# BaeHann/feature_level_style_transfer_for_TSC

Hardware: AMD Instinct MI355X
Metric: train-step samples/sec (univariate TS, len=512, batch=256) at 1/2/4/8 MI355X (higher is better)
Workload: dtype bf16x3

## Files before the change

### feature_level_style_transfer_for_tsc_amd/_lib.py

```python
from __future__ import annotations

import ctypes
import os
from ctypes import POINTER, Structure, c_char_p, c_float, c_int, c_int32, c_int64, c_void_p
from typing import Optional

import torch

ABI_VERSION = 13
_LIB_NAME = "libfst_hip.so"
_HERE = os.path.dirname(os.path.abspath(__file__))
LIB_PATH = os.environ.get("FST_HIP_LIB", os.path.join(_HERE, _LIB_NAME))


class FstLibraryError(RuntimeError):
    pass


class WSrc(Structure):
    _fields_ = [("w", c_void_p), ("off0", c_int64), ("sm", c_int64), ("sc", c_int64), ("st", c_int64)]


_P = c_void_p
_I32P = c_void_p
_SIGNATURES = {
    "fst_version": (c_int, []),
    "fst_last_error": (c_char_p, []),
    "fst_pack_weights": (c_int, [_I32P, _I32P, c_int, POINTER(WSrc), POINTER(WSrc), c_int, c_int, c_int, c_int, _P, c_void_p]),
    "fst_pack_weights_bf16x3": (c_int, [_I32P, _I32P, c_int, POINTER(WSrc), POINTER(WSrc), c_int, c_int, c_int, c_int, _P, c_void_p]),
    "fst_unpack_weights": (c_int, [_I32P, _I32P, c_int, _P, c_int, _P, c_int64, c_int64, c_int64, c_int64,
                                   _P, c_int64, c_int64, c_int64, c_int64, c_int, c_void_p]),
    "fst_mask_taps": (c_int, [_P, _I32P, _I32P, c_int, c_int, c_int, c_void_p]),
    "fst_conv_gemm": (c_int, [_P, c_int64, _P, c_int64, _P, _I32P, _I32P, c_int, _P, _P, c_int64, _P, c_int64,
                              _P, c_int64, c_int, c_int, c_int, c_int, c_int, c_int, c_int, c_int, c_void_p]),
    "fst_conv_wgrad": (c_int, [_P, c_int64, _P, c_int64, _P, c_int64, _P, c_int64, c_int, _P, _I32P, _I32P, c_int,
                               c_int, c_int, c_int, c_int, c_int, c_int64, c_void_p]),
    "fst_conv_last_route": (c_int, [POINTER(c_int32)]),
    "fst_row_sum": (c_int, [_P, c_int64, c_int, c_int, c_int, _P, c_void_p]),
    "fst_bn_stats": (c_int, [_P, c_int, c_int, c_int, _P, c_int64, c_void_p]),
    "fst_bn_finalize": (c_int, [_P, c_int, _P, _P, _P, _P, c_int, c_int, c_float, c_float, _P, c_void_p]),
    "fst_bn_apply": (c_int, [_P, _P, _P, _P, _P, c_int, c_int, c_int, c_int, c_int64, c_void_p]),
    "fst_bn_bwd_reduce": (c_int, [_P, _P, _P, _P, c_int, c_int, c_int, c_int, _P, c_int64, c_void_p]),
    "fst_bn_bwd_apply": (c_int, [_P, _P, _P, _P, _P, c_int, _P, _P, _P, c_int, c_int, c_int, c_int, c_int, c_int, c_int64, c_void_p]),
    "fst_gate_fwd": (c_int, [_P, _P, c_int, c_int, c_int, c_int64, c_void_p]),
    "fst_gate_bwd": (c_int, [_P, _P, _P, c_int, c_int, c_int, c_int64, c_void_p]),
    "fst_coupling_sum_slots": (c_int64, [c_int, c_int, c_int]),
    "fst_coupling_fwd": (c_int, [_P, _P, _P, c_int, c_int, c_int, c_int64, _P, c_void_p]),
    "fst_coupling_bwd": (c_int, [_P, _P, _P, _P, _P, _P, _P, _P, c_int, c_int, c_int, c_int64, c_void_p]),
    "fst_coupling_inv_fwd": (c_int, [_P, _P, _P, c_int, c_int, c_int, c_int64, c_void_p]),
    "fst_coupling_inv_bwd": (c_int, [_P, _P, _P, _P, _P, c_int, c_int, c_int, c_int64, c_void_p]),
    "fst_rmsprop_multi": (c_int, [_P, _P, _P, _P, _P, c_int, c_float, c_float, c_void_p]),
    "fst_adam_multi": (c_int, [_P, _P, _P, _P, _P, c_int, _P, c_float, c_float, c_float, c_float, c_void_p]),
    "fst_wn_stack_fwd_ok": (c_int, [c_int, c_int, c_int, c_int]),
    "fst_wn_stack_fwd": (c_int, [_P, _P, _P, c_int64, _P, _P, _P, c_int64, _P, c_int, c_int, c_int, c_int, c_int, c_int64, c_void_p]),
    "fst_wn_stack_bwd_ok": (c_int, [c_int, c_int, c_int, c_int]),
    "fst_wn_stack_bwd": (c_int, [_P, _P, _P, _P, _P, _P, _P, _P, _P, c_int64, c_int, c_int, c_int, c_int, c_int, c_int64, c_void_p]),
    "fst_wn_wgrad_ok": (c_int, [c_int, c_int, c_int, c_int, c_int, c_int]),
    "fst_wn_wgrad_workspace_floats": (c_int64, [c_int, c_int, c_int, c_int, c_int, c_int]),
    "fst_wn_wgrad_in": (c_int, [_P, _P, _P, c_int, c_int64, _P, _P, _P, c_int64, c_int, c_int, c_int, c_int, c_int, c_int, c_int64,
                                c_void_p]),
    "fst_wn_wgrad_rs": (c_int, [_P, _P, _P, c_int, _P, _P, c_int64, c_int, c_int, c_int, c_int, c_int64, c_void_p]),
    "fst_nt_gemm_workspace_floats": (c_int64, [c_int, c_int, c_int]),
    "fst_nt_gemm": (c_int, [_P, _P, _P, _P, c_int64, c_int, c_int, c_int, _P, _P, c_int, c_float, _P, c_void_p]),
    "fst_tap_wgrad_ok": (c_int, [c_int, c_int, c_int, c_int, c_int, c_int, c_int]),
    "fst_tap_wgrad_workspace_floats": (c_int64, [c_int, c_int, c_int, c_int, c_int]),
    "fst_tap_wgrad": (c_int, [_P, _P, _P, _P, c_int64, c_int, c_int, c_int, c_int, c_int, c_int, c_int, c_int, c_int64, c_int64, c_void_p]),
    "fst_dense_tap_wgrad_ok": (c_int, [c_int, c_int, c_int, c_int, c_int, c_int]),
    "fst_dense_tap_wgrad_workspace_floats": (c_int64, [c_int, c_int, c_int, c_int, c_int]),
    "fst_dense_tap_wgrad": (c_int, [_P, _P, _P, _P, c_int64, c_int, c_int, c_int, c_int, c_int, c_int, c_int64, c_int64, c_void_p]),
    "fst_relu_bwd": (c_int, [_P, _P, _P, c_int64, c_void_p]),
    "fst_gemm_workspace_floats": (c_int64, [c_int, c_int, c_int]),
    "fst_gemm": (c_int, [_P, c_int64, c_int, _P, c_int64, c_int, _P, c_int64, c_int, c_int, c_int, _P, c_int, c_float, _P, c_int64,
                         c_void_p]),
    "fst_act_bwd": (c_int, [_P, _P, _P, c_int64, c_float, c_void_p]),
    "fst_batch_sum": (c_int, [_P, _P, _P, c_int, c_int64, c_int, c_void_p]),
    "fst_noise_transfer_fwd": (c_int, [_P, c_int, c_int, _P, _P, c_float, c_float, _P, _P, _P, _P, _P, _P, _P, c_int, c_int, c_void_p]),
# ... 82 lines not shown
```

### feature_level_style_transfer_for_tsc_amd/csrc/pointwise.hip

```cpp
#include "fst_common.h"

static thread_local char g_err[512] = "";
void fst_set_error(const char* fmt, ...) {
  va_list ap;
  va_start(ap, fmt);
  vsnprintf(g_err, sizeof(g_err), fmt, ap);
  va_end(ap);
}
extern "C" const char* fst_last_error(void) { return g_err; }

int fst_allow_full_lds(const void* fn, const char* who) {
  static const void* done[64];
  static int n_done = 0;
  for (int i = 0; i < n_done; ++i)
    if (done[i] == fn) return 0;
  hipError_t e = hipFuncSetAttribute(fn, hipFuncAttributeMaxDynamicSharedMemorySize, 160 * 1024);
  if (e != hipSuccess) {
    fst_set_error("%s: hipFuncSetAttribute: %s", who, hipGetErrorString(e));
    return (int)e;
  }
  if (n_done < 64) done[n_done++] = fn;
  return 0;
}
int fst_cu_count(void) {
// ... 174 lines not shown
      const double nn = n + nb, d = mb - m;
      m += d * (nb / nn);
      m2 += Mb + d * d * (n * nb / nn);
      n = nn;
    }
    const double v = n > 0.0 ? m2 / n : 0.0;
    mean = (float)m;
    var = (float)v;
    const float unbiased = n > 1.0 ? (float)(m2 / (n - 1.0)) : var;
    rmean[c] = (1.f - momentum) * rmean[c] + momentum * mean;
    rvar[c] = (1.f - momentum) * rvar[c] + momentum * unbiased;
  } else {
    mean = rmean[c];
    var = rvar[c];
  }
  const float invstd = 1.0f / sqrtf(var + eps);
  const float scale = gamma[c] * invstd;
  stats[c] = mean;
  stats[C + c] = invstd;
  stats[2 * C + c] = scale;
  stats[3 * C + c] = beta[c] - mean * scale;
}

extern "C" int fst_bn_finalize(const float* part, int n_slots, const float* gamma, const float* beta, float* running_mean,
                               float* running_var, int train, int C, float eps, float momentum, float* stats, void* stream) {
  FST_REQUIRE(gamma && beta && running_mean && running_var && stats && C > 0, "fst_bn_finalize: bad arguments");
  FST_REQUIRE(!train || (part && n_slots > 0), "fst_bn_finalize: train mode needs the moment partials (n_slots=%d)", n_slots);
  hipLaunchKernelGGL(bn_finalize_kernel, dim3((C + 63) / 64), dim3(64), 0, (hipStream_t)stream, part, n_slots, gamma, beta,
                     running_mean, running_var, train, C, eps, momentum, stats);
  FST_LAUNCH_CHECK();
  return 0;
}

__global__ __launch_bounds__(256) void bn_apply_kernel(const float* y, const float* stats, const float* res,
                                                       const float* res_stats, float* out, int C, int L, int relu) {
  const int bc = blockIdx.x;
  const int c = bc % C;
  const float sc = stats[2 * C + c], sh = stats[3 * C + c];
  float rsc = 1.f, rsh = 0.f;
  if (res && res_stats) { rsc = res_stats[2 * C + c]; rsh = res_stats[3 * C + c]; }
  const long long base = (long long)bc * L;
  for (int t = threadIdx.x; t < L; t += 256) {
    float v = y[base + t] * sc + sh;
    if (res) v += res[base + t] * rsc + rsh;
    if (relu) v = fmaxf(v, 0.f);
    out[base + t] = v;
  }
}

__global__ __launch_bounds__(256) void bn_apply_vec_kernel(const float* y, const float* stats, const float* res,
                                                           const float* res_stats, float* out, int rows, int C, int L,
                                                           int relu, RowVec rv) {
  const int r = threadIdx.x >> rv.shift, t0 = threadIdx.x & ((1 << rv.shift) - 1), rpp = 256 >> rv.shift;
  const int bc = blockIdx.x * rpp + r;
  if (bc >= rows) return;
  const int c = bc % C;
  const float sc = stats[2 * C + c], sh = stats[3 * C + c];
  float rsc = 1.f, rsh = 0.f;
  if (res && res_stats) { rsc = res_stats[2 * C + c]; rsh = res_stats[3 * C + c]; }
  const long long base = (long long)bc * rv.L4;
  const float4* y4 = reinterpret_cast<const float4*>(y) + base;
  const float4* r4 = res ? reinterpret_cast<const float4*>(res) + base : nullptr;
  float4* o4 = reinterpret_cast<float4*>(out) + base;
  for (int t = t0; t < rv.L4; t += 1 << rv.shift) {
    float4 v = y4[t];
    v.x = v.x * sc + sh; v.y = v.y * sc + sh; v.z = v.z * sc + sh; v.w = v.w * sc + sh;
    if (r4) {
      const float4 q = r4[t];
      v.x += q.x * rsc + rsh; v.y += q.y * rsc + rsh; v.z += q.z * rsc + rsh; v.w += q.w * rsc + rsh;
    }
    if (relu) { v.x = fmaxf(v.x, 0.f); v.y = fmaxf(v.y, 0.f); v.z = fmaxf(v.z, 0.f); v.w = fmaxf(v.w, 0.f); }
    o4[t] = v;
  }
}

extern "C" int fst_bn_apply(const float* y, const float* stats, const float* res, const float* res_stats, float* out,
                            int B, int C, int L, int relu, int64_t numel, void* stream) {
  FST_REQUIRE(y && stats && out && B > 0 && C > 0 && L > 0, "fst_bn_apply: bad arguments");
  FST_REQUIRE_EXTENT("fst_bn_apply", B, C, L, numel);
  if (vec_ok(L, {y, res, out})) {
    const RowVec rv = row_vec(L);
    const int rpp = 256 >> rv.shift;
    hipLaunchKernelGGL(bn_apply_vec_kernel, dim3((B * C + rpp - 1) / rpp), dim3(256), 0, (hipStream_t)stream, y, stats, res,
                       res_stats, out, B * C, C, L, relu, rv);
  } else {
    hipLaunchKernelGGL(bn_apply_kernel, dim3(B * C), dim3(256), 0, (hipStream_t)stream, y, stats, res, res_stats, out, C, L, relu);
  }
  FST_LAUNCH_CHECK();
  return 0;
}

__global__ __launch_bounds__(256) void bn_bwd_reduce_kernel(const float* dy, const float* y, const float* out,
                                                            const float* stats, int B, int C, int L, int relu, float* red) {
  const int c = blockIdx.x;
  const float mean = stats[c], invstd = stats[C + c];
  float s1 = 0.f, s2 = 0.f;
  for (int b = blockIdx.y; b < B; b += gridDim.y) {
    const long long base = ((long long)b * C + c) * L;
    for (int t = threadIdx.x; t < L; t += 256) {
      float g = dy[base + t];
      if (relu && !(out[base + t] > 0.f)) g = 0.f;
      s1 += g;
// ... 54 lines not shown
}

__device__ __forceinline__ void bn_red_sums(const float* red, int n_slots, int C, int c, float& r1, float& r2) {
  r1 = 0.f; r2 = 0.f;
  for (int s = 0; s < n_slots; ++s) {
    r1 += red[(long long)c * n_slots + s];
    r2 += red[((long long)C + c) * n_slots + s];
  }
}

__global__ __launch_bounds__(256) void bn_bwd_apply_kernel(const float* dy, const float* y, const float* out,
                                                           const float* stats, const float* red, int n_slots, float* red_out,
                                                           float* dx, float* row_sums, int C, int L, int relu, int train, float invN) {
  const int bc = blockIdx.x;
  const int c = bc % C;
  const float mean = stats[c], invstd = stats[C + c], scale = stats[2 * C + c];
  float r1 = 0.f, r2 = 0.f;
  if (red) bn_red_sums(red, n_slots, C, c, r1, r2);
  if (red_out && bc < C && threadIdx.x == 0) { red_out[c] = r1; red_out[C + c] = r2; }
  const float m1 = train ? r1 * invN : 0.f, m2 = train ? r2 * invN : 0.f;
  const long long base = (long long)bc * L;
  float rs = 0.f, dummy = 0.f;
  for (int t = threadIdx.x; t < L; t += 256) {
    float g = dy[base + t];
    if (relu && !(out[base + t] > 0.f)) g = 0.f;
    const float xh = (y[base + t] - mean) * invstd;
    const float d = scale * (g - m1 - xh * m2);
    dx[base + t] = d;
    rs += d;
  }
  if (row_sums) {
    block_sum2(rs, dummy);
    if (threadIdx.x == 0) row_sums[bc] = rs;
  }
}

__global__ __launch_bounds__(256) void bn_bwd_apply_vec_kernel(const float* dy, const float* y, const float* out,
                                                               const float* stats, const float* red, int n_slots,
                                                               float* red_out, float* dx, float* row_sums, int rows, int C,
                                                               int L, int relu, int train, float invN, RowVec rv) {
  __shared__ float wsum[4];
  const int r = threadIdx.x >> rv.shift, t0 = threadIdx.x & ((1 << rv.shift) - 1), rpp = 256 >> rv.shift;
  const int bc_raw = blockIdx.x * rpp + r;
  const bool live = bc_raw < rows;
  const int bc = live ? bc_raw : rows - 1;
  const int c = bc % C;
  const float mean = stats[c], invstd = stats[C + c], scale = stats[2 * C + c];
  float r1 = 0.f, r2 = 0.f;
  if (red) bn_red_sums(red, n_slots, C, c, r1, r2);
  if (red_out && live && bc < C && t0 == 0) { red_out[c] = r1; red_out[C + c] = r2; }
  const float m1 = train ? r1 * invN : 0.f, m2 = train ? r2 * invN : 0.f;
  const long long base = (long long)bc * rv.L4;
  const float4* dy4 = reinterpret_cast<const float4*>(dy) + base;
  const float4* y4 = reinterpret_cast<const float4*>(y) + base;
  const float4* o4 = reinterpret_cast<const float4*>(out) + base;
  float4* dx4 = reinterpret_cast<float4*>(dx) + base;
  float rs = 0.f;
  for (int t = t0; t < rv.L4; t += 1 << rv.shift) {
    float4 g = dy4[t];
    const float4 v = y4[t];
    if (relu) {
      const float4 o = o4[t];
      if (!(o.x > 0.f)) g.x = 0.f;
      if (!(o.y > 0.f)) g.y = 0.f;
      if (!(o.z > 0.f)) g.z = 0.f;
      if (!(o.w > 0.f)) g.w = 0.f;
    }
    float4 d;
    d.x = scale * (g.x - m1 - (v.x - mean) * invstd * m2);
    d.y = scale * (g.y - m1 - (v.y - mean) * invstd * m2);
    d.z = scale * (g.z - m1 - (v.z - mean) * invstd * m2);
    d.w = scale * (g.w - m1 - (v.w - mean) * invstd * m2);
    if (live) dx4[t] = d;
    rs += (d.x + d.y) + (d.z + d.w);
  }
  if (row_sums) {
    const int w = rv.shift < 6 ? rv.shift : 6;
    for (int o = (1 << w) >> 1; o > 0; o >>= 1) rs += __shfl_xor(rs, o, 64);
    if (rv.shift <= 6) {
      if (live && t0 == 0) row_sums[bc] = rs;
    } else {
      if ((threadIdx.x & 63) == 0) wsum[threadIdx.x >> 6] = rs;
      __syncthreads();
      if (live && t0 == 0) {
        const int w0 = threadIdx.x >> 6, nw = 1 << (rv.shift - 6);
        float tot = 0.f;
        for (int i = 0; i < nw; ++i) tot += wsum[w0 + i];
        row_sums[bc] = tot;
      }
    }
  }
}

extern "C" int fst_bn_bwd_apply(const float* dy, const float* y, const float* out, const float* stats, const float* red,
                                int n_slots, float* red_out, float* dx, float* row_sums, int B, int C, int L, int relu, int train,
                                int B_total, int64_t numel, void* stream) {
  FST_REQUIRE(dy && y && stats && dx && (!relu || out) && (!train || red), "fst_bn_bwd_apply: bad arguments");
  FST_REQUIRE(B > 0 && C > 0 && L > 0 && B_total >= B, "fst_bn_bwd_apply: B=%d C=%d L=%d B_total=%d", B, C, L, B_total);
  FST_REQUIRE(!red || n_slots > 0, "fst_bn_bwd_apply: n_slots=%d", n_slots);
  FST_REQUIRE(!red_out || red, "fst_bn_bwd_apply: red_out needs red");
  FST_REQUIRE_EXTENT("fst_bn_bwd_apply", B, C, L, numel);
  if (vec_ok(L, {dy, y, out, dx})) {
    const RowVec rv = row_vec(L);
    const int rpp = 256 >> rv.shift;
    hipLaunchKernelGGL(bn_bwd_apply_vec_kernel, dim3((B * C + rpp - 1) / rpp), dim3(256), 0, (hipStream_t)stream, dy, y, out,
                       stats, red, n_slots, red_out, dx, row_sums, B * C, C, L, relu, train, 1.0f / ((float)B_total * (float)L), rv);
  } else {
    hipLaunchKernelGGL(bn_bwd_apply_kernel, dim3(B * C), dim3(256), 0, (hipStream_t)stream, dy, y, out, stats, red, n_slots,
                       red_out, dx, row_sums, C, L, relu, train, 1.0f / ((float)B_total * (float)L));
  }
  FST_LAUNCH_CHECK();
  return 0;
}

__global__ __launch_bounds__(256) void gate_fwd_kernel(float* g, float* acts, int n, int L) {
  const int b = blockIdx.y;
  const long long total = (long long)n * L;
  float* gt = g + (long long)b * 2 * total;
  float* gs = gt + total;
  float* ab = acts + (long long)b * total;
  for (long long i = (long long)blockIdx.x * 256 + threadIdx.x; i < total; i += (long long)gridDim.x * 256) {
    const float t = tanhf(gt[i]);
    const float s = 1.0f / (1.0f + expf(-gs[i]));
    gt[i] = t;
    gs[i] = s;
    ab[i] = t * s;
  }
}

extern "C" int fst_gate_fwd(float* g_ts, float* acts, int B, int n, int L, int64_t numel_acts, void* stream) {
  FST_REQUIRE(g_ts && acts && B > 0 && n > 0 && L > 0, "fst_gate_fwd: bad arguments");
  FST_REQUIRE_EXTENT("fst_gate_fwd", B, n, L, numel_acts);
  long long blocks = ((long long)n * L + 255) / 256;
  if (blocks > 64) blocks = 64;
  hipLaunchKernelGGL(gate_fwd_kernel, dim3((unsigned)blocks, B), dim3(256), 0, (hipStream_t)stream, g_ts, acts, n, L);
  FST_LAUNCH_CHECK();
  return 0;
}

__global__ __launch_bounds__(256) void gate_bwd_kernel(const float* ts, const float* dacts, float* dg, int n, int L) {
  const int b = blockIdx.y;
  const long long total = (long long)n * L;
  const float* tt = ts + (long long)b * 2 * total;
  const float* ss = tt + total;
  const float* da = dacts + (long long)b * total;
// ... 322 lines not shown
```

### feature_level_style_transfer_for_tsc_amd/ops.py

```python
from __future__ import annotations

import ctypes
import math
import os
from typing import Dict, List, Optional, Sequence, Tuple

import torch

from . import _lib
from . import dist as _dist
from ._lib import WSrc, check, ptr, stream_ptr
from .plan import Plan, Segment, build_plan, pick_mb

EPI_RELU, EPI_ACC2, EPI_ATOMIC, EPI_ACC1 = 1, 2, 4, 8
GEMM_BF16X3 = 16
WGRAD_SLABS = 32
MATH = os.environ.get("FST_MATH", "bf16x3")
LDS_BUDGET = 96 * 1024
LDS_MULTI_CHUNK = 44 * 1024
PIPE_C = 16

_PARTIAL_BACKWARD = False


# ... 626 lines not shown
        tag = getattr(dy, "_fst_row_sums", None)
        if tag is None or dy.dim() != 3:
            return None
        rs, version = tag
        if version != dy._version or tuple(rs.shape) != tuple(dy.shape[:2]) or not dy.is_contiguous():
            return None
        return rs


_ROW_SUMS = _RowSums()


def _bn_stats(y: Tensor, gamma: Tensor, beta: Tensor, rmean: Tensor, rvar: Tensor, training: bool, eps: float,
              momentum: float) -> Tensor:
    lib = _lib.load()
    B, C, L = y.shape
    stats = torch.empty(4 * C, device=y.device, dtype=torch.float32)
    part, n_slots = None, 0
    if training:
        part = torch.empty(C, BN_SLOTS, 4, device=y.device, dtype=torch.float32)
        check(lib.fst_bn_stats(ptr(y), B, C, L, ptr(part), y.numel(), stream_ptr()), "fst_bn_stats")
        part = _dist.gather_slots(part)
        n_slots = part.size(1)
    check(lib.fst_bn_finalize(ptr(part), n_slots, ptr(gamma), ptr(beta), ptr(rmean), ptr(rvar), int(training), C, eps,
                              momentum, ptr(stats), stream_ptr()), "fst_bn_finalize")
    return stats


def _bn_backward(dy: Tensor, y: Tensor, out: Optional[Tensor], stats: Tensor, relu: bool, training: bool,
                 need_dx: bool = True):
    lib = _lib.load()
    B, C, L = y.shape
    part = torch.empty(2, C, BN_SLOTS, device=y.device, dtype=torch.float32)
    check(lib.fst_bn_bwd_reduce(ptr(dy), ptr(y), ptr(out), ptr(stats), B, C, L, int(relu), ptr(part), _same_numel(dy, y, out),
                                stream_ptr()),
          "fst_bn_bwd_reduce")
    if not need_dx:
        red = part.sum(dim=2).view(2 * C)
        return None, red[C:], red[:C]
    dx = torch.empty_like(y)
    rs = torch.empty(B, C, device=y.device, dtype=torch.float32)
    if training and _dist.global_batch_active():
        red = part.sum(dim=2).view(2 * C)
        red_g = red.clone()
        B_total = _dist.sum_over_ranks_(red_g) * B
        check(lib.fst_bn_bwd_apply(ptr(dy), ptr(y), ptr(out), ptr(stats), ptr(red_g), 1, None, ptr(dx), ptr(rs), B, C, L, int(relu),
                                   int(training), B_total, _same_numel(dy, y, out, dx), stream_ptr()), "fst_bn_bwd_apply")
    else:
        red = torch.empty(2 * C, device=y.device, dtype=torch.float32)
        check(lib.fst_bn_bwd_apply(ptr(dy), ptr(y), ptr(out), ptr(stats), ptr(part), BN_SLOTS, ptr(red), ptr(dx), ptr(rs), B, C, L,
                                   int(relu), int(training), B, _same_numel(dy, y, out, dx), stream_ptr()), "fst_bn_bwd_apply")
    _ROW_SUMS.attach(dx, rs)
    return dx, red[C:], red[:C]


class BNActFn(torch.autograd.Function):

    @staticmethod
    def forward(ctx, y, gamma, beta, rmean, rvar, training: bool, relu: bool, eps: float, momentum: float):
        lib = _lib.load()
        y = y.contiguous()
        B, C, L = y.shape
        stats = _bn_stats(y, gamma, beta, rmean, rvar, training, eps, momentum)
        out = torch.empty_like(y)
        check(lib.fst_bn_apply(ptr(y), ptr(stats), None, None, ptr(out), B, C, L, int(relu), _same_numel(y, out), stream_ptr()),
              "fst_bn_apply")
        ctx.save_for_backward(y, out, stats)
        ctx.relu, ctx.training = relu, training
        return out

    @staticmethod
    def backward(ctx, dout):
        y, out, stats = ctx.saved_tensors
        dx, dg, db = _bn_backward(dout.contiguous(), y, out if ctx.relu else None, stats, ctx.relu, ctx.training,
                                  ctx.needs_input_grad[0])
        return dx, dg, db, None, None, None, None, None, None


class BNAddBNReluFn(torch.autograd.Function):

    @staticmethod
    def forward(ctx, ya, ga, ba, rma, rva, yb, gb, bb, rmb, rvb, training: bool, eps: float, momentum: float):
        lib = _lib.load()
        ya, yb = ya.contiguous(), yb.contiguous()
        B, C, L = ya.shape
        sa = _bn_stats(ya, ga, ba, rma, rva, training, eps, momentum)
        sb = _bn_stats(yb, gb, bb, rmb, rvb, training, eps, momentum)
        out = torch.empty_like(ya)
        check(lib.fst_bn_apply(ptr(ya), ptr(sa), ptr(yb), ptr(sb), ptr(out), B, C, L, 1, _same_numel(ya, yb, out), stream_ptr()),
              "fst_bn_apply")
        ctx.save_for_backward(ya, yb, out, sa, sb)
        ctx.training = training
        return out

    @staticmethod
    def backward(ctx, dout):
        ya, yb, out, sa, sb = ctx.saved_tensors
        dout = dout.contiguous()
        dxa, dga, dba = _bn_backward(dout, ya, out, sa, True, ctx.training, ctx.needs_input_grad[0])
        dxb, dgb, dbb = _bn_backward(dout, yb, out, sb, True, ctx.training, ctx.needs_input_grad[5])
        return dxa, dga, dba, None, None, dxb, dgb, dbb, None, None, None, None, None


class WNSpecs:

    def __init__(self, h: int, n: int, n_layers: int = 8, kernel: int = 3):
        self.h, self.n, self.n_layers, self.kernel = h, n, n_layers, kernel
        self.start = ConvSpec(n, h)
        self.ins = [ConvSpec(2 * n, n, kernel, 2 ** i, int((kernel * 2 ** i - 2 ** i) / 2), C1=h) for i in range(n_layers)]
        self.rs = [ConvSpec(2 * n if i < n_layers - 1 else n, n) for i in range(n_layers)]
        self.end = ConvSpec(2 * h, n)
        self.rs_T = build_plan(n, [Segment(0, n, 0, 1), Segment(1, n, 0, 1)], 1, 1, 0, chunk_c=PIPE_C)
        self.rs_T_last = build_plan(n, [Segment(0, n, 0, 1)], 1, 1, 0, chunk_c=PIPE_C)
        nl = n_layers
        self.shapes = ([(n, h, 1), (n,), (2 * n * nl, h, 1), (2 * n * nl,), (2 * h, n, 1), (2 * h,)]
                       + [(2 * n, n, kernel)] * nl + [(2 * n,)] * nl
                       + [(2 * n if i < nl - 1 else n, n, 1) for i in range(nl)] + [(2 * n if i < nl - 1 else n,) for i in range(nl)])
        self.offsets = [0]
        for sh in self.shapes:
            self.offsets.append(self.offsets[-1] + int(math.prod(sh)))
        self.flat_numel = self.offsets[-1]

    def flatten(self, weights: Sequence[Tensor]) -> Tensor:
        assert len(weights) == len(self.shapes) and all(tuple(w.shape) == sh for w, sh in zip(weights, self.shapes))
        return torch.cat([w.reshape(-1) for w in weights])

    def unflatten(self, flat: Tensor) -> List[Tensor]:
        assert flat.numel() == self.flat_numel and flat.is_contiguous()
        return [flat[self.offsets[i]: self.offsets[i + 1]].view(sh) for i, sh in enumerate(self.shapes)]


def wn_wgrad_ok(kind: int, B: int, L: int, n: int, h: int, dil: int, a: Optional[Tensor] = None) -> bool:
    if MATH != "bf16x3" or os.environ.get("FST_WN_WGRAD", "1") == "0":
# ... 1100 lines not shown
```

### include/fst_hip.h

```cpp
#ifndef FST_HIP_H
#define FST_HIP_H

#include <stdint.h>

#ifdef __cplusplus
extern "C" {
#endif

#define FST_ABI_VERSION 13

int fst_version(void);
const char* fst_last_error(void);

#define FST_PLAN_HEADER 16

typedef struct {
  const float* w;
  int64_t off0, sm, sc, st;
} fst_wsrc;

int fst_pack_weights(const int32_t* plan_dev, const int32_t* plan_host, int plan_len,
                     const fst_wsrc* src0_host, const fst_wsrc* src1_host,
                     int M, int g_begin, int g_end , int row_base ,
                     float* a_packed, void* stream);

int fst_pack_weights_bf16x3(const int32_t* plan_dev, const int32_t* plan_host, int plan_len,
                            const fst_wsrc* src0_host, const fst_wsrc* src1_host,
                            int M, int g_begin, int g_end, int row_base, void* a_image, void* stream);

int fst_unpack_weights(const int32_t* plan_dev, const int32_t* plan_host, int plan_len,
                       const float* a_packed, int M,
                       float* dw0, int64_t off0_0, int64_t sm0, int64_t sc0, int64_t st0,
                       float* dw1, int64_t off0_1, int64_t sm1, int64_t sc1, int64_t st1,
                       int n_slabs ,
                       void* stream);

int fst_mask_taps(float* w, const int32_t* live_lo, const int32_t* live_hi, int M, int C, int K, void* stream);

#define FST_EPI_RELU    1
#define FST_EPI_ACC2    2
#define FST_EPI_ATOMIC  4
#define FST_EPI_ACC1    8
// ... 8 lines not shown

int fst_conv_wgrad(const float* x0, int64_t x0_bs, const float* x1, int64_t x1_bs,
                   const float* dy, int64_t dy_bs, const float* dy2, int64_t dy2_bs, int msplit,
                   float* da_packed, const int32_t* plan_dev, const int32_t* plan_host, int plan_len,
                   int B, int L, int M, int ksplit, int flags , int64_t x0_mul_off, void* stream);

#define FST_ROUTE_GEMM      1
#define FST_ROUTE_PIPE      2
#define FST_ROUTE_BF3       3
#define FST_ROUTE_WIN_BF3   4
#define FST_ROUTE_WIN_ROWS  5
#define FST_ROUTE_WGRAD     6
#define FST_ROUTE_EPI_PLAIN   0
#define FST_ROUTE_EPI_ADD     1
#define FST_ROUTE_EPI_ATOMIC  2
#define FST_ROUTE_EPI_VEC     3
#define FST_ROUTE_EPI_VEC_ADD 4
int fst_conv_last_route(int32_t out[8]);

int fst_row_sum(const float* x, int64_t x_bs, int B, int C, int L, float* out, void* stream);

#define FST_BN_SLOTS 16
int fst_bn_stats(const float* y, int B, int C, int L, float* part , int64_t numel, void* stream);
int fst_bn_finalize(const float* part, int n_slots, const float* gamma, const float* beta,
                    float* running_mean, float* running_var, int train, int C, float eps, float momentum,
                    float* stats, void* stream);
int fst_bn_apply(const float* y, const float* stats, const float* res, const float* res_stats,
                 float* out, int B, int C, int L, int relu, int64_t numel, void* stream);
int fst_bn_bwd_reduce(const float* dy, const float* y, const float* out, const float* stats,
                      int B, int C, int L, int relu, float* red , int64_t numel, void* stream);
int fst_bn_bwd_apply(const float* dy, const float* y, const float* out, const float* stats, const float* red, int n_slots,
                     float* red_out, float* dx, float* row_sums, int B, int C, int L, int relu, int train, int B_total,
                     int64_t numel, void* stream);

int fst_gate_fwd(float* g_ts, float* acts, int B, int n, int L, int64_t numel_acts, void* stream);
int fst_gate_bwd(const float* ts, const float* dacts, float* dg, int B, int n, int L, int64_t numel_acts, void* stream);
int64_t fst_coupling_sum_slots(int B, int h, int L);
int fst_coupling_fwd(const float* u, const float* o, float* xn, int B, int h, int L, int64_t numel, float* sums, void* stream);
int fst_coupling_bwd(const float* u, const float* o, const float* dxn, const float* dlogs, const float* g_ls, const float* g_sq,
                     float* du, float* d_o, int B, int h, int L, int64_t numel, void* stream);
int fst_coupling_inv_fwd(const float* x, const float* o, float* xn, int B, int h, int L, int64_t numel, void* stream);
int fst_coupling_inv_bwd(const float* xn, const float* o, const float* dxn,
                         float* dx, float* d_o, int B, int h, int L, int64_t numel, void* stream);

int fst_wn_fold_fwd(const int64_t* table_dev, int n_rows, float* flat, float* norms , void* stream);
int fst_wn_fold_bwd(const int64_t* table_dev, int n_rows, const float* d_flat, const float* norms, float* dpar, void* stream);

int fst_logdet_inv(const float* W, int n, float* out , float* inv_t , void* stream);

int64_t fst_wn_image_bytes(int n, int h);
int fst_wn_pack(const float* in_w, const float* cond_w, const float* in_b, const float* cond_b,
                const float* rs_w, const float* rs_b, int n, int h, int ntaps , int last, void* image, int64_t image_bytes, void* stream);
int fst_wn_layer_fwd(const float* a, int64_t a_bs, const float* u0, int64_t u0_bs, const void* image, int64_t image_bytes,
                     float* ts, float* acts, float* a_next, float* out, int first, int last,
                     int B, int L, int n, int h, int dil, int64_t numel_a, void* stream);

int64_t fst_wn_bwd_image_bytes(int n, int last);
int fst_wn_pack_bwd(const float* rs_w, int n, int last,
                    int acc_order ,
                    void* image, int64_t image_bytes, void* stream);
int fst_wn_layer_bwd(const float* d_a_next , const float* d_out, const float* ts, const void* image,
                     int64_t image_bytes, float* dg,
                     float* row_sums ,
                     int64_t row_sums_rows, int last, int B, int L, int n, int64_t numel_a, void* stream);

int64_t fst_wn_dgrad_image_bytes(int n);
// ... 99 lines not shown
```

Measured before the change: 3474.

## Recompute ReLU mask from BN inputs and fuse dual-branch BN backward

BN+ReLU backward now rebuilds the ReLU mask from the pre-BN input and per-channel stats instead of reading the saved forward output, so the output tensor is no longer kept for backward. The residual-join BN backward runs both branches in one reduce kernel and one apply kernel, reading dout once instead of twice and cutting launches. This lowers memory traffic and activation memory at the cost of a few extra FMAs per element. The recomputed mask can differ from the forward output in rare rounding cases near zero.

```diff
diff --git a/feature_level_style_transfer_for_tsc_amd/_lib.py b/feature_level_style_transfer_for_tsc_amd/_lib.py
--- a/feature_level_style_transfer_for_tsc_amd/_lib.py
+++ b/feature_level_style_transfer_for_tsc_amd/_lib.py
@@ -7,7 +7,7 @@
 
 import torch
 
-ABI_VERSION = 13
+ABI_VERSION = 14
 _LIB_NAME = "libfst_hip.so"
 _HERE = os.path.dirname(os.path.abspath(__file__))
 LIB_PATH = os.environ.get("FST_HIP_LIB", os.path.join(_HERE, _LIB_NAME))
@@ -42,6 +42,11 @@
     "fst_bn_apply": (c_int, [_P, _P, _P, _P, _P, c_int, c_int, c_int, c_int, c_int64, c_void_p]),
     "fst_bn_bwd_reduce": (c_int, [_P, _P, _P, _P, c_int, c_int, c_int, c_int, _P, c_int64, c_void_p]),
     "fst_bn_bwd_apply": (c_int, [_P, _P, _P, _P, _P, c_int, _P, _P, _P, c_int, c_int, c_int, c_int, c_int, c_int, c_int64, c_void_p]),
+    "fst_bn_relu_bwd_reduce": (c_int, [_P, _P, _P, c_int, c_int, c_int, _P, c_int64, c_void_p]),
+    "fst_bn_relu_bwd_apply": (c_int, [_P, _P, _P, _P, c_int, _P, _P, _P, c_int, c_int, c_int, c_int, c_int, c_int64, c_void_p]),
+    "fst_bn_join_bwd_reduce": (c_int, [_P, _P, _P, _P, _P, c_int, c_int, c_int, _P, _P, c_int64, c_void_p]),
+    "fst_bn_join_bwd_apply": (c_int, [_P, _P, _P, _P, _P, _P, _P, _P, _P, _P, _P, _P, _P, c_int, c_int, c_int, c_int, c_int, c_int,
+                                      c_int64, c_void_p]),
     "fst_gate_fwd": (c_int, [_P, _P, c_int, c_int, c_int, c_int64, c_void_p]),
     "fst_gate_bwd": (c_int, [_P, _P, _P, c_int, c_int, c_int, c_int64, c_void_p]),
     "fst_coupling_sum_slots": (c_int64, [c_int, c_int, c_int]),
diff --git a/feature_level_style_transfer_for_tsc_amd/csrc/pointwise.hip b/feature_level_style_transfer_for_tsc_amd/csrc/pointwise.hip
--- a/feature_level_style_transfer_for_tsc_amd/csrc/pointwise.hip
+++ b/feature_level_style_transfer_for_tsc_amd/csrc/pointwise.hip
@@ -230,6 +230,9 @@
   return 0;
 }
 
+__device__ __forceinline__ float bn_affine(float y, float sc, float sh) { return fmaf(y, sc, sh); }
+__device__ __forceinline__ float bn_affine_add(float v, float res, float rsc, float rsh) { return v + fmaf(res, rsc, rsh); }
+
 __global__ __launch_bounds__(256) void bn_apply_kernel(const float* y, const float* stats, const float* res,
                                                        const float* res_stats, float* out, int C, int L, int relu) {
   const int bc = blockIdx.x;
@@ -239,8 +242,8 @@
   if (res && res_stats) { rsc = res_stats[2 * C + c]; rsh = res_stats[3 * C + c]; }
   const long long base = (long long)bc * L;
   for (int t = threadIdx.x; t < L; t += 256) {
-    float v = y[base + t] * sc + sh;
-    if (res) v += res[base + t] * rsc + rsh;
+    float v = bn_affine(y[base + t], sc, sh);
+    if (res) v = bn_affine_add(v, res[base + t], rsc, rsh);
     if (relu) v = fmaxf(v, 0.f);
     out[base + t] = v;
   }
@@ -262,10 +265,11 @@
   float4* o4 = reinterpret_cast<float4*>(out) + base;
   for (int t = t0; t < rv.L4; t += 1 << rv.shift) {
     float4 v = y4[t];
-    v.x = v.x * sc + sh; v.y = v.y * sc + sh; v.z = v.z * sc + sh; v.w = v.w * sc + sh;
+    v.x = bn_affine(v.x, sc, sh); v.y = bn_affine(v.y, sc, sh); v.z = bn_affine(v.z, sc, sh); v.w = bn_affine(v.w, sc, sh);
     if (r4) {
       const float4 q = r4[t];
-      v.x += q.x * rsc + rsh; v.y += q.y * rsc + rsh; v.z += q.z * rsc + rsh; v.w += q.w * rsc + rsh;
+      v.x = bn_affine_add(v.x, q.x, rsc, rsh); v.y = bn_affine_add(v.y, q.y, rsc, rsh);
+      v.z = bn_affine_add(v.z, q.z, rsc, rsh); v.w = bn_affine_add(v.w, q.w, rsc, rsh);
     }
     if (relu) { v.x = fmaxf(v.x, 0.f); v.y = fmaxf(v.y, 0.f); v.z = fmaxf(v.z, 0.f); v.w = fmaxf(v.w, 0.f); }
     o4[t] = v;
@@ -386,6 +390,24 @@
   if (row_sums) {
     block_sum2(rs, dummy);
     if (threadIdx.x == 0) row_sums[bc] = rs;
+  }
+}
+
+__device__ __forceinline__ void bn_store_row_sum(float rs, const RowVec& rv, bool live, int t0, int bc, float* row_sums,
+                                                 float* wsum) {
+  const int w = rv.shift < 6 ? rv.shift : 6;
+  for (int o = (1 << w) >> 1; o > 0; o >>= 1) rs += __shfl_xor(rs, o, 64);
+  if (rv.shift <= 6) {
+    if (live && t0 == 0) row_sums[bc] = rs;
+  } else {
+    if ((threadIdx.x & 63) == 0) wsum[threadIdx.x >> 6] = rs;
+    __syncthreads();
+    if (live && t0 == 0) {
+      const int w0 = threadIdx.x >> 6, nw = 1 << (rv.shift - 6);
+      float tot = 0.f;
+      for (int i = 0; i < nw; ++i) tot += wsum[w0 + i];
+      row_sums[bc] = tot;
+    }
   }
 }
 
@@ -428,22 +450,7 @@
     if (live) dx4[t] = d;
     rs += (d.x + d.y) + (d.z + d.w);
   }
-  if (row_sums) {
-    const int w = rv.shift < 6 ? rv.shift : 6;
-    for (int o = (1 << w) >> 1; o > 0; o >>= 1) rs += __shfl_xor(rs, o, 64);
-    if (rv.shift <= 6) {
-      if (live && t0 == 0) row_sums[bc] = rs;
-    } else {
-      if ((threadIdx.x & 63) == 0) wsum[threadIdx.x >> 6] = rs;
-      __syncthreads();
-      if (live && t0 == 0) {
-        const int w0 = threadIdx.x >> 6, nw = 1 << (rv.shift - 6);
-        float tot = 0.f;
-        for (int i = 0; i < nw; ++i) tot += wsum[w0 + i];
-        row_sums[bc] = tot;
-      }
-    }
-  }
+  if (row_sums) bn_store_row_sum(rs, rv, live, t0, bc, row_sums, wsum);
 }
 
 extern "C" int fst_bn_bwd_apply(const float* dy, const float* y, const float* out, const float* stats, const float* red,
@@ -465,6 +472,281 @@
   }
   FST_LAUNCH_CHECK();
   return 0;
+}
+
+template <int NB>
+struct BnMaskReduceArgs {
+  const float* y[NB];
+  const float* stats[NB];
+  float* red[NB];
+};
+template <int NB>
+struct BnMaskApplyArgs {
+  const float* y[NB];
+  const float* stats[NB];
+  const float* red[NB];
+  float* red_out[NB];
+  float* dx[NB];
+  float* row_sums[NB];
+};
+
+template <int NB>
+__device__ __forceinline__ bool bn_out_positive(float ya, float yb, const float* sc, const float* sh) {
+  float v = bn_affine(ya, sc[0], sh[0]);
+  if (NB == 2) v = bn_affine_add(v, yb, sc[1], sh[1]);
+  return v > 0.f;
+}
+
+template <int NB>
+__device__ __forceinline__ void bn_mask_store_slot(float s1, float* s2, const BnMaskReduceArgs<NB>& a, int C, int c) {
+  float unused = 0.f;
+  block_sum2(s1, s2[0]);
+  if (NB == 2) block_sum2(unused, s2[1]);
+  if (threadIdx.x == 0) {
+#pragma unroll
+    for (int i = 0; i < NB; ++i) {
+      a.red[i][(long long)c * FST_BN_SLOTS + blockIdx.y] = s1;
+      a.red[i][((long long)C + c) * FST_BN_SLOTS + blockIdx.y] = s2[i];
+    }
+  }
+}
+
+template <int NB>
+__global__ __launch_bounds__(256) void bn_mask_bwd_reduce_kernel(const float* dy, BnMaskReduceArgs<NB> a, int B, int C, int L) {
+  const int c = blockIdx.x;
+  float mean[NB], invstd[NB], sc[NB], sh[NB], s2[NB];
+#pragma unroll
+  for (int i = 0; i < NB; ++i) {
+    mean[i] = a.stats[i][c]; invstd[i] = a.stats[i][C + c]; sc[i] = a.stats[i][2 * C + c]; sh[i] = a.stats[i][3 * C + c];
+    s2[i] = 0.f;
+  }
+  float s1 = 0.f;
+  for (int b = blockIdx.y; b < B; b += gridDim.y) {
+    const long long base = ((long long)b * C + c) * L;
+    for (int t = threadIdx.x; t < L; t += 256) {
+      float g = dy[base + t];
+      float v[NB];
+#pragma unroll
+      for (int i = 0; i < NB; ++i) v[i] = a.y[i][base + t];
+      if (!bn_out_positive<NB>(v[0], v[NB - 1], sc, sh)) g = 0.f;
+      s1 += g;
+#pragma unroll
+      for (int i = 0; i < NB; ++i) s2[i] += g * (v[i] - mean[i]) * invstd[i];
+    }
+  }
+  bn_mask_store_slot<NB>(s1, s2, a, C, c);
+}
+
+template <int NB>
+__global__ __launch_bounds__(256) void bn_mask_bwd_reduce_vec_kernel(const float* dy, BnMaskReduceArgs<NB> a, int B, int C, int L,
+                                                                     RowVec rv) {
+  const int c = blockIdx.x, r = threadIdx.x >> rv.shift, t0 = threadIdx.x & ((1 << rv.shift) - 1), rpp = 256 >> rv.shift;
+  float mean[NB], invstd[NB], sc[NB], sh[NB], s2[NB];
+#pragma unroll
+  for (int i = 0; i < NB; ++i) {
+    mean[i] = a.stats[i][c]; invstd[i] = a.stats[i][C + c]; sc[i] = a.stats[i][2 * C + c]; sh[i] = a.stats[i][3 * C + c];
+    s2[i] = 0.f;
+  }
+  float s1 = 0.f;
+  for (int b = blockIdx.y + r * gridDim.y; b < B; b += rpp * gridDim.y) {
+    const long long base = ((long long)b * C + c) * rv.L4;
+    const float4* dy4 = reinterpret_cast<const float4*>(dy) + base;
+    const float4* y4[NB];
+#pragma unroll
+    for (int i = 0; i < NB; ++i) y4[i] = reinterpret_cast<const float4*>(a.y[i]) + base;
+    for (int t = t0; t < rv.L4; t += 1 << rv.shift) {
+      float4 g = dy4[t];
+      float4 v[NB];
+#pragma unroll
+      for (int i = 0; i < NB; ++i) v[i] = y4[i][t];
+      if (!bn_out_positive<NB>(v[0].x, v[NB - 1].x, sc, sh)) g.x = 0.f;
+      if (!bn_out_positive<NB>(v[0].y, v[NB - 1].y, sc, sh)) g.y = 0.f;
+      if (!bn_out_positive<NB>(v[0].z, v[NB - 1].z, sc, sh)) g.z = 0.f;
+      if (!bn_out_positive<NB>(v[0].w, v[NB - 1].w, sc, sh)) g.w = 0.f;
+      s1 += (g.x + g.y) + (g.z + g.w);
+#pragma unroll
+      for (int i = 0; i < NB; ++i)
+        s2[i] += (g.x * (v[i].x - mean[i]) + g.y * (v[i].y - mean[i]) + g.z * (v[i].z - mean[i]) + g.w * (v[i].w - mean[i])) * invstd[i];
+    }
+  }
+  bn_mask_store_slot<NB>(s1, s2, a, C, c);
+}
+
+template <int NB>
+static int launch_bn_mask_bwd_reduce(const char* who, const float* dy, const BnMaskReduceArgs<NB>& a, int B, int C, int L,
+                                     int64_t numel, void* stream) {
+  bool ok = dy && B > 0 && C > 0 && L > 0;
+  for (int i = 0; i < NB; ++i) ok = ok && a.y[i] && a.stats[i] && a.red[i];
+  FST_REQUIRE(ok, "%s: bad arguments", who);
+  FST_REQUIRE_EXTENT(who, B, C, L, numel);
+  if (vec_ok(L, {dy, a.y[0], a.y[NB - 1]}))
+    hipLaunchKernelGGL(bn_mask_bwd_reduce_vec_kernel<NB>, dim3(C, FST_BN_SLOTS), dim3(256), 0, (hipStream_t)stream, dy, a, B, C, L,
+                       row_vec(L));
+  else
+    hipLaunchKernelGGL(bn_mask_bwd_reduce_kernel<NB>, dim3(C, FST_BN_SLOTS), dim3(256), 0, (hipStream_t)stream, dy, a, B, C, L);
+  FST_LAUNCH_CHECK();
+  return 0;
+}
+
+extern "C" int fst_bn_relu_bwd_reduce(const float* dy, const float* y, const float* stats, int B, int C, int L, float* red,
+                                      int64_t numel, void* stream) {
+  const BnMaskReduceArgs<1> a = {{y}, {stats}, {red}};
+  return launch_bn_mask_bwd_reduce<1>("fst_bn_relu_bwd_reduce", dy, a, B, C, L, numel, stream);
+}
+
+extern "C" int fst_bn_join_bwd_reduce(const float* dout, const float* ya, const float* stats_a, const float* yb,
+                                      const float* stats_b, int B, int C, int L, float* red_a, float* red_b, int64_t numel,
+                                      void* stream) {
+  const BnMaskReduceArgs<2> a = {{ya, yb}, {stats_a, stats_b}, {red_a, red_b}};
+  return launch_bn_mask_bwd_reduce<2>("fst_bn_join_bwd_reduce", dout, a, B, C, L, numel, stream);
+}
+
+struct BnBranchCoef {
+  float mean, invstd, scale, m1, m2;
+};
+template <int NB>
+__device__ __forceinline__ void bn_mask_apply_coefs(const BnMaskApplyArgs<NB>& a, int n_slots, int C, int c, bool first_row,
+                                                    int train, float invN, BnBranchCoef* k, float* sc, float* sh) {
+#pragma unroll
+  for (int i = 0; i < NB; ++i) {
+    k[i].mean = a.stats[i][c]; k[i].invstd = a.stats[i][C + c]; k[i].scale = a.stats[i][2 * C + c];
+    sc[i] = k[i].scale; sh[i] = a.stats[i][3 * C + c];
+    float r1 = 0.f, r2 = 0.f;
+    if (a.red[i]) bn_red_sums(a.red[i], n_slots, C, c, r1, r2);
+    if (a.red_out[i] && first_row) { a.red_out[i][c] = r1; a.red_out[i][C + c] = r2; }
+    k[i].m1 = train ? r1 * invN : 0.f;
+    k[i].m2 = train ? r2 * invN : 0.f;
+  }
+}
+
+template <int NB>
+__global__ __launch_bounds__(256) void bn_mask_bwd_apply_kernel(const float* dy, BnMaskApplyArgs<NB> a, int n_slots, int C, int L,
+                                                                int train, float invN) {
+  const int bc = blockIdx.x;
+  const int c = bc % C;
+  BnBranchCoef k[NB];
+  float sc[NB], sh[NB], rs[NB];
+  bn_mask_apply_coefs<NB>(a, n_slots, C, c, bc < C && threadIdx.x == 0, train, invN, k, sc, sh);
+#pragma unroll
+  for (int i = 0; i < NB; ++i) rs[i] = 0.f;
+  const long long base = (long long)bc * L;
+  for (int t = threadIdx.x; t < L; t += 256) {
+    float g = dy[base + t];
+    float v[NB];
+#pragma unroll
+    for (int i = 0; i < NB; ++i) v[i] = a.y[i][base + t];
+    if (!bn_out_positive<NB>(v[0], v[NB - 1], sc, sh)) g = 0.f;
+#pragma unroll
+    for (int i = 0; i < NB; ++i) {
+      if (!a.dx[i]) continue;
+      const float xh = (v[i] - k[i].mean) * k[i].invstd;
+      const float d = k[i].scale * (g - k[i].m1 - xh * k[i].m2);
+      a.dx[i][base + t] = d;
+      rs[i] += d;
+    }
+  }
+#pragma unroll
+  for (int i = 0; i < NB; ++i) {
+    if (a.dx[i] && a.row_sums[i]) {
+      float dummy = 0.f;
+      block_sum2(rs[i], dummy);
+      if (threadIdx.x == 0) a.row_sums[i][bc] = rs[i];
+    }
+  }
+}
+
+template <int NB>
+__global__ __launch_bounds__(256) void bn_mask_bwd_apply_vec_kernel(const float* dy, BnMaskApplyArgs<NB> a, int n_slots, int rows,
+                                                                    int C, int L, int train, float invN, RowVec rv) {
+  __shared__ float wsum[NB][4];
+  const int r = threadIdx.x >> rv.shift, t0 = threadIdx.x & ((1 << rv.shift) - 1), rpp = 256 >> rv.shift;
+  const int bc_raw = blockIdx.x * rpp + r;
+  const bool live = bc_raw < rows;
+  const int bc = live ? bc_raw : rows - 1;
+  const int c = bc % C;
+  BnBranchCoef k[NB];
+  float sc[NB], sh[NB], rs[NB];
+  bn_mask_apply_coefs<NB>(a, n_slots, C, c, live && bc < C && t0 == 0, train, invN, k, sc, sh);
+  const long long base = (long long)bc * rv.L4;
+  const float4* dy4 = reinterpret_cast<const float4*>(dy) + base;
+  const float4* y4[NB];
+  float4* dx4[NB];
+#pragma unroll
+  for (int i = 0; i < NB; ++i) {
+    y4[i] = reinterpret_cast<const float4*>(a.y[i]) + base;
+    dx4[i] = a.dx[i] ? reinterpret_cast<float4*>(a.dx[i]) + base : nullptr;
+    rs[i] = 0.f;
+  }
+  for (int t = t0; t < rv.L4; t += 1 << rv.shift) {
+    float4 g = dy4[t];
+    float4 v[NB];
+#pragma unroll
+    for (int i = 0; i < NB; ++i) v[i] = y4[i][t];
+    if (!bn_out_positive<NB>(v[0].x, v[NB - 1].x, sc, sh)) g.x = 0.f;
+    if (!bn_out_positive<NB>(v[0].y, v[NB - 1].y, sc, sh)) g.y = 0.f;
+    if (!bn_out_positive<NB>(v[0].z, v[NB - 1].z, sc, sh)) g.z = 0.f;
+    if (!bn_out_positive<NB>(v[0].w, v[NB - 1].w, sc, sh)) g.w = 0.f;
+#pragma unroll
+    for (int i = 0; i < NB; ++i) {
+      if (!dx4[i]) continue;
+      const float mean = k[i].mean, invstd = k[i].invstd, scale = k[i].scale, m1 = k[i].m1, m2 = k[i].m2;
+      float4 d;
+      d.x = scale * (g.x - m1 - (v[i].x - mean) * invstd * m2);
+      d.y = scale * (g.y - m1 - (v[i].y - mean) * invstd * m2);
+      d.z = scale * (g.z - m1 - (v[i].z - mean) * invstd * m2);
+      d.w = scale * (g.w - m1 - (v[i].w - mean) * invstd * m2);
+      if (live) dx4[i][t] = d;
+      rs[i] += (d.x + d.y) + (d.z + d.w);
+    }
+  }
+#pragma unroll
+  for (int i = 0; i < NB; ++i)
+    if (dx4[i] && a.row_sums[i]) bn_store_row_sum(rs[i], rv, live, t0, bc, a.row_sums[i], wsum[i]);
+}
+
+template <int NB>
+static int launch_bn_mask_bwd_apply(const char* who, const float* dy, const BnMaskApplyArgs<NB>& a, int n_slots, int B, int C,
+                                    int L, int train, int B_total, int64_t numel, void* stream) {
+  bool ok = dy != nullptr, any_dx = false;
+  for (int i = 0; i < NB; ++i) {
+    ok = ok && a.y[i] && a.stats[i] && (!train || a.red[i]);
+    any_dx = any_dx || a.dx[i];
+  }
+  FST_REQUIRE(ok && any_dx, "%s: bad arguments", who);
+  FST_REQUIRE(B > 0 && C > 0 && L > 0 && B_total >= B, "%s: B=%d C=%d L=%d B_total=%d", who, B, C, L, B_total);
+  for (int i = 0; i < NB; ++i) {
+    FST_REQUIRE(!a.red[i] || n_slots > 0, "%s: n_slots=%d", who, n_slots);
+    FST_REQUIRE(!a.red_out[i] || a.red[i], "%s: red_out needs red", who);
+  }
+  FST_REQUIRE_EXTENT(who, B, C, L, numel);
+  const float invN = 1.0f / ((float)B_total * (float)L);
+  if (vec_ok(L, {dy, a.y[0], a.y[NB - 1], a.dx[0], a.dx[NB - 1]})) {
+    const RowVec rv = row_vec(L);
+    const int rpp = 256 >> rv.shift;
+    hipLaunchKernelGGL(bn_mask_bwd_apply_vec_kernel<NB>, dim3((B * C + rpp - 1) / rpp), dim3(256), 0, (hipStream_t)stream, dy, a,
+                       n_slots, B * C, C, L, train, invN, rv);
+  } else {
+    hipLaunchKernelGGL(bn_mask_bwd_apply_kernel<NB>, dim3(B * C), dim3(256), 0, (hipStream_t)stream, dy, a, n_slots, C, L, train,
+                       invN);
+  }
+  FST_LAUNCH_CHECK();
+  return 0;
+}
+
+extern "C" int fst_bn_relu_bwd_apply(const float* dy, const float* y, const float* stats, const float* red, int n_slots,
+                                     float* red_out, float* dx, float* row_sums, int B, int C, int L, int train, int B_total,
+                                     int64_t numel, void* stream) {
+  const BnMaskApplyArgs<1> a = {{y}, {stats}, {red}, {red_out}, {dx}, {row_sums}};
+  return launch_bn_mask_bwd_apply<1>("fst_bn_relu_bwd_apply", dy, a, n_slots, B, C, L, train, B_total, numel, stream);
+}
+
+extern "C" int fst_bn_join_bwd_apply(const float* dout, const float* ya, const float* stats_a, const float* red_a,
+                                     float* red_out_a, float* dxa, float* row_sums_a, const float* yb, const float* stats_b,
+                                     const float* red_b, float* red_out_b, float* dxb, float* row_sums_b, int n_slots, int B,
+                                     int C, int L, int train, int B_total, int64_t numel, void* stream) {
+  const BnMaskApplyArgs<2> a = {{ya, yb}, {stats_a, stats_b}, {red_a, red_b}, {red_out_a, red_out_b}, {dxa, dxb},
+                                {row_sums_a, row_sums_b}};
+  return launch_bn_mask_bwd_apply<2>("fst_bn_join_bwd_apply", dout, a, n_slots, B, C, L, train, B_total, numel, stream);
 }
 
 __global__ __launch_bounds__(256) void gate_fwd_kernel(float* g, float* acts, int n, int L) {
diff --git a/feature_level_style_transfer_for_tsc_amd/ops.py b/feature_level_style_transfer_for_tsc_amd/ops.py
--- a/feature_level_style_transfer_for_tsc_amd/ops.py
+++ b/feature_level_style_transfer_for_tsc_amd/ops.py
@@ -682,9 +682,12 @@
     lib = _lib.load()
     B, C, L = y.shape
     part = torch.empty(2, C, BN_SLOTS, device=y.device, dtype=torch.float32)
-    check(lib.fst_bn_bwd_reduce(ptr(dy), ptr(y), ptr(out), ptr(stats), B, C, L, int(relu), ptr(part), _same_numel(dy, y, out),
-                                stream_ptr()),
-          "fst_bn_bwd_reduce")
+    if relu:
+        check(lib.fst_bn_relu_bwd_reduce(ptr(dy), ptr(y), ptr(stats), B, C, L, ptr(part), _same_numel(dy, y), stream_ptr()),
+              "fst_bn_relu_bwd_reduce")
+    else:
+        check(lib.fst_bn_bwd_reduce(ptr(dy), ptr(y), None, ptr(stats), B, C, L, 0, ptr(part), _same_numel(dy, y), stream_ptr()),
+              "fst_bn_bwd_reduce")
     if not need_dx:
         red = part.sum(dim=2).view(2 * C)
         return None, red[C:], red[:C]
@@ -692,16 +695,50 @@
     rs = torch.empty(B, C, device=y.device, dtype=torch.float32)
     if training and _dist.global_batch_active():
         red = part.sum(dim=2).view(2 * C)
-        red_g = red.clone()
-        B_total = _dist.sum_over_ranks_(red_g) * B
-        check(lib.fst_bn_bwd_apply(ptr(dy), ptr(y), ptr(out), ptr(stats), ptr(red_g), 1, None, ptr(dx), ptr(rs), B, C, L, int(relu),
-                                   int(training), B_total, _same_numel(dy, y, out, dx), stream_ptr()), "fst_bn_bwd_apply")
+        red_in = red.clone()
+        n_slots, red_out, B_total = 1, None, _dist.sum_over_ranks_(red_in) * B
     else:
         red = torch.empty(2 * C, device=y.device, dtype=torch.float32)
-        check(lib.fst_bn_bwd_apply(ptr(dy), ptr(y), ptr(out), ptr(stats), ptr(part), BN_SLOTS, ptr(red), ptr(dx), ptr(rs), B, C, L,
-                                   int(relu), int(training), B, _same_numel(dy, y, out, dx), stream_ptr()), "fst_bn_bwd_apply")
+        red_in, n_slots, red_out, B_total = part, BN_SLOTS, red, B
+    if relu:
+        check(lib.fst_bn_relu_bwd_apply(ptr(dy), ptr(y), ptr(stats), ptr(red_in), n_slots, ptr(red_out), ptr(dx), ptr(rs), B, C, L,
+                                        int(training), B_total, _same_numel(dy, y, dx), stream_ptr()), "fst_bn_relu_bwd_apply")
+    else:
+        check(lib.fst_bn_bwd_apply(ptr(dy), ptr(y), None, ptr(stats), ptr(red_in), n_slots, ptr(red_out), ptr(dx), ptr(rs), B, C, L,
+                                   0, int(training), B_total, _same_numel(dy, y, dx), stream_ptr()), "fst_bn_bwd_apply")
     _ROW_SUMS.attach(dx, rs)
     return dx, red[C:], red[:C]
+
+
+def _bn_join_backward(dout: Tensor, ya: Tensor, sa: Tensor, yb: Tensor, sb: Tensor, training: bool, need_a: bool, need_b: bool):
+    lib = _lib.load()
+    B, C, L = ya.shape
+    part = torch.empty(2, 2, C, BN_SLOTS, device=ya.device, dtype=torch.float32)
+    check(lib.fst_bn_join_bwd_reduce(ptr(dout), ptr(ya), ptr(sa), ptr(yb), ptr(sb), B, C, L, ptr(part[0]), ptr(part[1]),
+                                     _same_numel(dout, ya, yb), stream_ptr()), "fst_bn_join_bwd_reduce")
+    if not (need_a or need_b):
+        red = part.sum(dim=3).view(2, 2 * C)
+        return None, red[0, C:], red[0, :C], None, red[1, C:], red[1, :C]
+    dxa = torch.empty_like(ya) if need_a else None
+    dxb = torch.empty_like(yb) if need_b else None
+    rsa = torch.empty(B, C, device=ya.device, dtype=torch.float32) if need_a else None
+    rsb = torch.empty(B, C, device=ya.device, dtype=torch.float32) if need_b else None
+    if training and _dist.global_batch_active():
+        red = part.sum(dim=3).view(2, 2 * C)
+        red_in = red.clone()
+        n_slots, red_out, B_total = 1, (None, None), _dist.sum_over_ranks_(red_in) * B
+    else:
+        red = torch.empty(2, 2 * C, device=ya.device, dtype=torch.float32)
+        red_in, n_slots, red_out, B_total = part, BN_SLOTS, red, B
+    check(lib.fst_bn_join_bwd_apply(ptr(dout), ptr(ya), ptr(sa), ptr(red_in[0]), ptr(red_out[0]), ptr(dxa), ptr(rsa),
+                                    ptr(yb), ptr(sb), ptr(red_in[1]), ptr(red_out[1]), ptr(dxb), ptr(rsb), n_slots, B, C, L,
+                                    int(training), B_total, _same_numel(dout, ya, yb, dxa, dxb), stream_ptr()),
+          "fst_bn_join_bwd_apply")
+    if need_a:
+        _ROW_SUMS.attach(dxa, rsa)
+    if need_b:
+        _ROW_SUMS.attach(dxb, rsb)
+    return dxa, red[0, C:], red[0, :C], dxb, red[1, C:], red[1, :C]
 
 
 class BNActFn(torch.autograd.Function):
@@ -715,15 +752,14 @@
         out = torch.empty_like(y)
         check(lib.fst_bn_apply(ptr(y), ptr(stats), None, None, ptr(out), B, C, L, int(relu), _same_numel(y, out), stream_ptr()),
               "fst_bn_apply")
-        ctx.save_for_backward(y, out, stats)
+        ctx.save_for_backward(y, stats)
         ctx.relu, ctx.training = relu, training
         return out
 
     @staticmethod
     def backward(ctx, dout):
-        y, out, stats = ctx.saved_tensors
-        dx, dg, db = _bn_backward(dout.contiguous(), y, out if ctx.relu else None, stats, ctx.relu, ctx.training,
-                                  ctx.needs_input_grad[0])
+        y, stats = ctx.saved_tensors
+        dx, dg, db = _bn_backward(dout.contiguous(), y, None, stats, ctx.relu, ctx.training, ctx.needs_input_grad[0])
         return dx, dg, db, None, None, None, None, None, None
 
 
@@ -739,16 +775,15 @@
         out = torch.empty_like(ya)
         check(lib.fst_bn_apply(ptr(ya), ptr(sa), ptr(yb), ptr(sb), ptr(out), B, C, L, 1, _same_numel(ya, yb, out), stream_ptr()),
               "fst_bn_apply")
-        ctx.save_for_backward(ya, yb, out, sa, sb)
+        ctx.save_for_backward(ya, yb, sa, sb)
         ctx.training = training
         return out
 
     @staticmethod
     def backward(ctx, dout):
-        ya, yb, out, sa, sb = ctx.saved_tensors
-        dout = dout.contiguous()
-        dxa, dga, dba = _bn_backward(dout, ya, out, sa, True, ctx.training, ctx.needs_input_grad[0])
-        dxb, dgb, dbb = _bn_backward(dout, yb, out, sb, True, ctx.training, ctx.needs_input_grad[5])
+        ya, yb, sa, sb = ctx.saved_tensors
+        dxa, dga, dba, dxb, dgb, dbb = _bn_join_backward(dout.contiguous(), ya, sa, yb, sb, ctx.training, ctx.needs_input_grad[0],
+                                                         ctx.needs_input_grad[5])
         return dxa, dga, dba, None, None, dxb, dgb, dbb, None, None, None, None, None
 
 
diff --git a/include/fst_hip.h b/include/fst_hip.h
--- a/include/fst_hip.h
+++ b/include/fst_hip.h
@@ -7,7 +7,7 @@
 extern "C" {
 #endif
 
-#define FST_ABI_VERSION 13
+#define FST_ABI_VERSION 14
 
 int fst_version(void);
 const char* fst_last_error(void);
@@ -82,6 +82,17 @@
 int fst_bn_bwd_apply(const float* dy, const float* y, const float* out, const float* stats, const float* red, int n_slots,
                      float* red_out, float* dx, float* row_sums, int B, int C, int L, int relu, int train, int B_total,
                      int64_t numel, void* stream);
+int fst_bn_relu_bwd_reduce(const float* dy, const float* y, const float* stats, int B, int C, int L,
+                           float* red , int64_t numel, void* stream);
+int fst_bn_relu_bwd_apply(const float* dy, const float* y, const float* stats, const float* red, int n_slots, float* red_out,
+                          float* dx, float* row_sums, int B, int C, int L, int train, int B_total, int64_t numel, void* stream);
+int fst_bn_join_bwd_reduce(const float* dout, const float* ya, const float* stats_a, const float* yb, const float* stats_b,
+                           int B, int C, int L, float* red_a, float* red_b , int64_t numel,
+                           void* stream);
+int fst_bn_join_bwd_apply(const float* dout, const float* ya, const float* stats_a, const float* red_a, float* red_out_a,
+                          float* dxa, float* row_sums_a, const float* yb, const float* stats_b, const float* red_b,
+                          float* red_out_b, float* dxb, float* row_sums_b, int n_slots, int B, int C, int L, int train,
+                          int B_total, int64_t numel, void* stream);
 
 int fst_gate_fwd(float* g_ts, float* acts, int B, int n, int L, int64_t numel_acts, void* stream);
 int fst_gate_bwd(const float* ts, const float* dacts, float* dg, int B, int n, int L, int64_t numel_acts, void* stream);
```

Result: no change. 3501, median of 6 (+0.8%).
